# alexbuburuzan/MObI

Hardware: AMD Instinct MI355X
Metric: denoising throughput (UNet element-forwards/s = steps/s x UNet batch) (higher is better)
Workload: dtype bf16; 1 GPU; mobi_nusc_512 UNet denoising step, 8 objects/GPU (UNet batch 16), latent 64x64, DDIM-50 schedule, cfg_scale 1.0; objects_per_gpu=8, unet_batch=16, latent=64, sampler=ddim, parallelism=dp1 (objects sharded, no collective in the loop)

## Files before the change

### include/mobi_engine.h

```cpp
#ifndef MOBI_ENGINE_H_
#define MOBI_ENGINE_H_

#include <stddef.h>
#include <stdint.h>

#ifdef __cplusplus
extern "C" {
#endif

#define MOBI_ABI_VERSION 6

enum { MOBI_OK = 0, MOBI_ERR_ARG = -1, MOBI_ERR_UNSUPPORTED = -2, MOBI_ERR_LAUNCH = -3, MOBI_ERR_ALIGN = -4 };
enum { MOBI_F16 = 0, MOBI_BF16 = 1 };

int mobi_abi_version(void);
const char* mobi_error_string(int code);
size_t mobi_struct_size(int id);
int mobi_tuning_reload(void);
int mobi_build_info(void);

enum { MOBI_EPI_NONE = 0, MOBI_EPI_GEGLU = 1, MOBI_EPI_LEAKY_RELU = 2 };
enum { MOBI_OUT_ROWS = 0,
       MOBI_OUT_TRANSPOSED = 1,
       MOBI_OUT_ROWS_F32 = 2 };

typedef struct mobi_igemm_params {
  const void* src0;
  const void* src1;
  int32_t c0, c1;
  int32_t batch;
  int32_t hin, win;
  int32_t upsample;
  int32_t hout, wout;
  int32_t kh, kw, stride, pad_h, pad_w;
  int64_t src_img_stride;
  const void* weight;
  int32_t groups;
  int64_t w_group_stride;
  int32_t n_packed;
  int32_t cout;
  const float* bias;
  const float* rowvec;
  int32_t rowvec_stride;
  const void* residual;
  int64_t res_img_stride;
  void* out;
  int64_t out_img_stride;
  int32_t out_mode;
  int32_t epilogue;
  float scale;
  int32_t dtype;
  int32_t split_k;
  void* ws;
  int32_t k_order;
  const void* weight_tiled;
  void* sync;
  const float* ln_svec;
  float ln_eps;
  int32_t defer_finish;
} mobi_igemm_params;

int mobi_igemm(const mobi_igemm_params* p, void* stream);
int32_t mobi_igemm_slab_count(const mobi_igemm_params* p);
int mobi_igemm_finish(const mobi_igemm_params* p, void* stream);
int mobi_igemm_plan_splits(const mobi_igemm_params* p);
enum { MOBI_IGEMM_STAGED_128 = 0, MOBI_IGEMM_STAGED_256 = 1, MOBI_IGEMM_DIRECT_LDS = 2, MOBI_IGEMM_PINGPONG = 3,
       MOBI_IGEMM_RING_128 = 4, MOBI_IGEMM_RING_256 = 5, MOBI_IGEMM_RING_128W = 6, MOBI_IGEMM_SMALL = 7 };
int mobi_igemm_kernel_variant(const mobi_igemm_params* p);
size_t mobi_igemm_workspace_bytes(const mobi_igemm_params* p, int32_t splits);
size_t mobi_igemm_sync_bytes(const mobi_igemm_params* p, int32_t splits);

typedef struct mobi_split_source {
  const float* slabs;
  int32_t count;
  int32_t row_stride;
  const float* bias;
  const float* rowvec;
  int32_t rowvec_stride;
  const void* residual;
  int64_t res_img_stride;
  void* finished;
} mobi_split_source;

typedef struct mobi_groupnorm_params {
  const void* src0;
  const void* src1;
  int32_t c0, c1;
  int32_t batch, hw;
  const float* gamma;
  const float* beta;
  float eps;
  int32_t silu;
  void* out;
  void* ws;
  int32_t dtype;
  int32_t src_f32;
  int32_t out_mode;
  void* sync;
  const mobi_split_source* src0_split;
} mobi_groupnorm_params;

size_t mobi_groupnorm_workspace_bytes(int32_t batch, int32_t hw);
int mobi_groupnorm_takes_split(int32_t c0, int32_t c1, int32_t batch, int32_t hw);
int mobi_groupnorm(const mobi_groupnorm_params* p, void* stream);

typedef struct mobi_layernorm_params {
  const void* src; void* out;
  int32_t images, rows_per_image, channels;
  int64_t src_img_stride, out_img_stride;
  const float* gamma; const float* beta; float eps;
  int32_t dtype;
} mobi_layernorm_params;
int mobi_layernorm(const mobi_layernorm_params* p, void* stream);

typedef struct mobi_attention_params {
  const void* q;  int64_t q_img_stride;  int32_t q_row_stride;
  const void* k;  int64_t k_img_stride;  int32_t k_row_stride;
  const void* vt; int64_t vt_img_stride; int32_t vt_row_stride;
  void* out;      int64_t out_img_stride; int32_t out_row_stride;
  int32_t images, heads, dh, tq, tk;
  float scale;
// ... 335 lines not shown
```

### mobi_amd/_lib.py

```python
import ctypes as C
import os

HERE = os.path.dirname(os.path.abspath(__file__))
LIB_PATH = os.path.join(HERE, "libmobi_hip.so")

MOBI_F16, MOBI_BF16 = 0, 1
ABI_VERSION = 6
EPI_NONE, EPI_GEGLU, EPI_LEAKY_RELU = 0, 1, 2
OUT_ROWS, OUT_TRANSPOSED, OUT_ROWS_F32 = 0, 1, 2
ACT_NONE, ACT_SILU, ACT_GELU = 0, 1, 2

vp, i32, i64, f32 = C.c_void_p, C.c_int32, C.c_int64, C.c_float


class EngineUnavailable(RuntimeError):
    pass


class EngineError(RuntimeError):
    pass


class IgemmParams(C.Structure):
    _fields_ = [("src0", vp), ("src1", vp), ("c0", i32), ("c1", i32), ("batch", i32), ("hin", i32), ("win", i32),
# ... 131 lines not shown
    _fields_ = [("frames", vp), ("corners_xy", vp), ("invert", vp), ("crop", vp), ("gt", vp), ("inpaint", vp), ("mask", vp),
                ("batch", i32), ("H", i32), ("W", i32), ("height", i32), ("width", i32)]


class LpipsDistanceParams(C.Structure):
    _fields_ = [("feat", vp), ("lin", vp), ("out", vp), ("ws", vp), ("pairs", i32), ("hw", i32), ("channels", i32), ("eps", f32),
                ("relu_in_place", i32), ("dtype", i32)]


class ImageNormalizeParams(C.Structure):
    _fields_ = [("src", vp), ("out", vp), ("batch", i32), ("channels", i32), ("hw", i32), ("shift", f32 * 4), ("scale", f32 * 4),
                ("nhwc_channels", i32), ("dtype", i32)]


class MtTensor(C.Structure):
    _fields_ = [("param", vp), ("grad", vp), ("exp_avg", vp), ("exp_avg_sq", vp), ("n", i64)]


class MtPair(C.Structure):
    _fields_ = [("a", vp), ("b", vp), ("n", i64)]


MT_EMA, MT_SWAP = 0, 1


class MtChunk(C.Structure):
    _fields_ = [("offset", i64), ("tensor", i32), ("reserved", i32)]


class GradStatsRecord(C.Structure):
    _fields_ = [("sumsq", C.c_double), ("nonfinite", i32), ("reserved", i32)]


STRUCT_IDS = {0: IgemmParams, 1: GroupNormParams, 2: LayerNormParams, 3: AttentionParams, 4: CtxAttentionParams,
              5: SkinnyLinearParams, 6: ConvSmallCinParams, 7: ConvSmallCoutParams, 8: DdimStepParams, 9: TwoKeyAdapterParams,
              10: RangePasteParams, 11: LidarMetricsParams, 12: RangePrepareParams, 13: ImagePrepareParams,
              14: FfGegluParams, 15: RowChainParams, 16: ChainOp,
              17: LayerNormBwdParams, 18: AttentionBwdParams, 19: SplitSource, 20: DpmStepParams,
              21: LpipsDistanceParams, 22: ImageNormalizeParams, 23: MtTensor, 24: MtChunk, 25: GradStatsRecord,
              26: MtPair}

SYMBOLS = {
    "mobi_abi_version": (C.c_int, []),
    "mobi_error_string": (C.c_char_p, [C.c_int]),
    "mobi_struct_size": (C.c_size_t, [C.c_int]),
    "mobi_tuning_reload": (C.c_int, []),
    "mobi_build_info": (C.c_int, []),
    "mobi_igemm": (C.c_int, [C.POINTER(IgemmParams), vp]),
    "mobi_igemm_plan_splits": (C.c_int, [C.POINTER(IgemmParams)]),
    "mobi_igemm_kernel_variant": (C.c_int, [C.POINTER(IgemmParams)]),
    "mobi_igemm_workspace_bytes": (C.c_size_t, [C.POINTER(IgemmParams), i32]),
    "mobi_igemm_sync_bytes": (C.c_size_t, [C.POINTER(IgemmParams), i32]),
    "mobi_igemm_slab_count": (i32, [C.POINTER(IgemmParams)]),
    "mobi_igemm_finish": (C.c_int, [C.POINTER(IgemmParams), vp]),
    "mobi_groupnorm_takes_split": (C.c_int, [i32, i32, i32, i32]),
    "mobi_groupnorm_workspace_bytes": (C.c_size_t, [i32, i32]),
    "mobi_groupnorm": (C.c_int, [C.POINTER(GroupNormParams), vp]),
    "mobi_layernorm": (C.c_int, [C.POINTER(LayerNormParams), vp]),
    "mobi_attention": (C.c_int, [C.POINTER(AttentionParams), vp]),
    "mobi_ctx_attention": (C.c_int, [C.POINTER(CtxAttentionParams), vp]),
    "mobi_two_key_adapter": (C.c_int, [C.POINTER(TwoKeyAdapterParams), vp]),
    "mobi_two_key_adapter_fuses_ln": (C.c_int, [i32, i64]),
    "mobi_softmax_rows": (C.c_int, [vp, vp, i64, i32, i32, vp]),
    "mobi_skinny_linear": (C.c_int, [C.POINTER(SkinnyLinearParams), vp]),
    "mobi_layernorm_rows_f32": (C.c_int, [vp, vp, vp, vp, i32, i32, i32, i32, f32, vp]),
    "mobi_linear_f32": (C.c_int, [vp, vp, vp, vp, i32, i32, i32, i32, i32, i32, vp]),
    "mobi_ff_geglu": (C.c_int, [C.POINTER(FfGegluParams), vp]),
    "mobi_ff_geglu_packed_bytes": (C.c_size_t, [i32, i32]),
    "mobi_row_chain": (C.c_int, [C.POINTER(RowChainParams), vp]),
    "mobi_groupnorm_scale_shift": (C.c_int, [vp, vp, vp, f32, vp, vp, i32, i32, i32, i32, vp]),
    "mobi_row_chain_weight_bytes": (C.c_size_t, [i32]),
    "mobi_row_chain_supported": (C.c_int, [i32, i32]),
    "mobi_row_chain_adapter_image_bytes": (C.c_size_t, [i32]),
    "mobi_row_chain_adapter_image": (C.c_int, [vp, vp, vp, vp, i32, i32, i32, i32, vp, vp]),
    "mobi_trunk_add": (C.c_int, [vp, vp, vp, i64, i32, vp]),
    "mobi_split_f32": (C.c_int, [vp, vp, i64, i32, i32, i32, vp]),
    "mobi_transpose": (C.c_int, [vp, i64, vp, i32, i32, i32, vp]),
    "mobi_tile_weights": (C.c_int, [vp, vp, i32, i32, vp]),
    "mobi_backward_partial_blocks": (i32, [i64]),
    "mobi_colsum": (C.c_int, [vp, i64, i64, i32, i32, vp, vp, vp]),
    "mobi_layernorm_bwd": (C.c_int, [C.POINTER(LayerNormBwdParams), vp]),
    "mobi_geglu_fwd": (C.c_int, [vp, vp, i64, i32, i32, vp]),
    "mobi_geglu_bwd": (C.c_int, [vp, vp, vp, i64, i32, i32, vp]),
    "mobi_attention_bwd": (C.c_int, [C.POINTER(AttentionBwdParams), vp]),
    "mobi_groupnorm_bwd_workspace_floats": (C.c_size_t, [i32, i32, i32]),
    "mobi_groupnorm_bwd": (C.c_int, [vp, vp, vp, vp, f32, i32, vp, vp, i32, i32, i32, i32, vp, vp]),
    "mobi_sumpool2": (C.c_int, [vp, vp, i32, i32, i32, i32, i32, vp]),
    "mobi_add": (C.c_int, [vp, vp, vp, i64, i32, vp]),
    "mobi_silu_bwd_f32": (C.c_int, [vp, vp, vp, i64, vp]),
    "mobi_adamw_step": (C.c_int, [vp, vp, vp, vp, i64, f32, f32, f32, f32, f32, i32, vp]),
    "mobi_multi_tensor_workspace_bytes": (C.c_size_t, [C.POINTER(i32)]),
    "mobi_grad_stats": (C.c_int, [vp, i32, vp, i32, vp, vp, vp]),
    "mobi_adamw_multi": (C.c_int, [vp, i32, vp, i32, f32, f32, f32, f32, f32, f32, i32, vp]),
    "mobi_ema_multi": (C.c_int, [vp, i32, vp, i32, f32, i32, vp]),
    "mobi_quick_gelu": (C.c_int, [vp, vp, i64, i32, vp]),
    "mobi_timestep_embedding": (C.c_int, [vp, vp, vp, i32, i32, vp]),
    "mobi_conv_small_cin": (C.c_int, [C.POINTER(ConvSmallCinParams), vp]),
    "mobi_conv_small_cout": (C.c_int, [C.POINTER(ConvSmallCoutParams), vp]),
    "mobi_ddim_step": (C.c_int, [C.POINTER(DdimStepParams), vp]),
    "mobi_dpm_step": (C.c_int, [C.POINTER(DpmStepParams), vp]),
    "mobi_lincomb4": (C.c_int, [vp, vp, vp, vp, vp, f32, f32, f32, f32, i64, vp]),
    "mobi_q_sample": (C.c_int, [vp, vp, vp, vp, vp, vp, i32, i32, i32, vp]),
    "mobi_mask_blend": (C.c_int, [vp, vp, vp, vp, f32, f32, i32, i32, i32, vp]),
    "mobi_posterior_sample": (C.c_int, [vp, vp, vp, i32, i32, i32, i32, i32, f32, vp]),
    "mobi_range_denorm": (C.c_int, [vp, vp, vp, f32, f32, f32, f32, i32, i32, vp, vp, i32, i32, vp]),
    "mobi_range_paste": (C.c_int, [C.POINTER(RangePasteParams), vp]),
# ... 57 lines not shown
```

### mobi_amd/csrc/igemm.hip

```cpp
#include <stdlib.h>

#include <type_traits>

#include "common.h"
#include "tuning.h"
#include "igemm_small.h"

#ifndef MOBI_FRAG2
#define MOBI_FRAG2 0
#endif
#ifndef MOBI_DMA_KS
#define MOBI_DMA_KS 1
#endif
#if defined(MOBI_IGEMM_FENCE) && MOBI_IGEMM_FENCE
#define MOBI_SCHED_FENCE() __builtin_amdgcn_sched_barrier(0)
#else
#define MOBI_SCHED_FENCE() ((void)0)
#endif

#ifndef MOBI_DBG_SKIP
#define MOBI_DBG_SKIP 0
#endif
#ifndef MOBI_PP_DMA_KS
#define MOBI_PP_DMA_KS 1
// ... 1639 lines not shown
#pragma unroll
  for (int i = 0; i < 4; ++i) {
    sum = __builtin_amdgcn_fdot2(q.p[i], one, sum, false);
    sq = __builtin_amdgcn_fdot2(q.p[i], q.p[i], sq, false);
  }
}
__device__ __forceinline__ void rowstat_acc(const bf16x8& x, float& sum, float& sq) {
  struct Q { bf16x2_t p[4]; };
  const Q q = __builtin_bit_cast(Q, x);
  const bf16x2_t one = {(__bf16)1.0f, (__bf16)1.0f};
#pragma unroll
  for (int i = 0; i < 4; ++i) {
    sum = __builtin_amdgcn_fdot2_f32_bf16(q.p[i], one, sum, false);
    sq = __builtin_amdgcn_fdot2_f32_bf16(q.p[i], q.p[i], sq, false);
  }
}

template <int NT, int MT, int SPW>
__device__ __forceinline__ void ln_fold_acc(const IgemmArgs& a, f32x4 (&acc)[NT][MT], const float (&ls_sum)[SPW],
                                            const float (&ls_sq)[SPW], float* s_rowstat, int lane, int wm, int wn, int nw0,
                                            bool add_bias) {
  const int r16 = lane & 15, g4 = lane >> 4;
  const float inv_k = 1.0f / (float)a.ktot;
#pragma unroll
  for (int i = 0; i < SPW; ++i) {
    float sm = ls_sum[i], sq = ls_sq[i];
    sm += __shfl_xor(sm, 16, 64); sq += __shfl_xor(sq, 16, 64);
    sm += __shfl_xor(sm, 32, 64); sq += __shfl_xor(sq, 32, 64);
    const float mean = sm * inv_k;
    const float var = fmaxf(sq * inv_k - mean * mean, 0.f);
    if (g4 == 0) {
      float* d = s_rowstat + ((wm * MT + SPW * wn + i) * 16 + r16) * 2;
      d[0] = mean; d[1] = rsqrtf(var + a.ln_eps);
    }
  }
  __syncthreads();
#pragma unroll
  for (int ni = 0; ni < NT; ++ni) {
    const int n = nw0 + ni * 16 + g4 * 4;
    f32x4 sv = f32x4{0.f, 0.f, 0.f, 0.f}, bv = f32x4{0.f, 0.f, 0.f, 0.f};
    if (n < a.n_packed) {
      sv = *reinterpret_cast<const f32x4*>(a.ln_svec + n);
      if (add_bias && a.bias) bv = *reinterpret_cast<const f32x4*>(a.bias + n);
    }
#pragma unroll
    for (int mi = 0; mi < MT; ++mi) {
      const float* d = s_rowstat + ((wm * MT + mi) * 16 + r16) * 2;
      const float mean = d[0], rstd = d[1];
      acc[ni][mi] = rstd * (acc[ni][mi] - mean * sv) + bv;
    }
  }
}

template <typename T, int NT, bool TR, int NW, int MT, bool LNF = false, bool LEAKY = false>
__global__ __launch_bounds__(NW * 64, 2) void igemm_ring_kernel(const IgemmArgs a) {
  typedef typename Vec8<T>::type frag_t;
  constexpr bool WIDE = NW == 8;
  constexpr int BM = 2 * MT * 16;
  constexpr int APW = BM / 16 / NW;
  constexpr int WAVE_N = NT * 16;
  constexpr int BN = (NW / 2) * WAVE_N;
  constexpr int WPIECES = BN / 16;
  constexpr int SLOT = (BM + BN) * 64;
  constexpr int RING = 4 * SLOT;
  constexpr int STAGE_BYTES = EpiGeom<32, TR, NT>::BYTES;
  constexpr int LDS_BYTES = RING > NW * STAGE_BYTES ? RING : NW * STAGE_BYTES;
  constexpr unsigned OOB = 0x80000000u;
  __shared__ __attribute__((aligned(16))) unsigned char lds[LDS_BYTES];
  __shared__ int s_arrive;
  __shared__ float s_rowstat[LNF ? BM * 2 : 2];
  static_assert(!(LNF && TR), "the LayerNorm fold has no transposed-output form");
  typedef __attribute__((address_space(3))) void* lds_ptr_t;

  const int tid = threadIdx.x, lane = tid & 63, wave = tid >> 6;
  const int wave_s = __builtin_amdgcn_readfirstlane(wave);
  const int wm = wave & 1, wn = wave >> 1;
  const int group = blockIdx.z;
  const int nblk = a.tiles_m * a.tiles_n;
  const int L = xcd_remap(blockIdx.x, nblk);
  MOBI_TILE_OF(L, tile_m, tile_n);
  const int m0 = tile_m * BM, n0 = tile_n * BN;
  constexpr int SPW = MT / (NW / 2);
  constexpr bool lnf = LNF;
  float ls_sum[SPW], ls_sq[SPW];
#pragma unroll
  for (int i = 0; i < SPW; ++i) ls_sum[i] = ls_sq[i] = 0.f;
  MOBI_STAMP_AT(0);
  const bool w_tiled = a.w_tiled != nullptr;
  const T* wgt = (w_tiled ? reinterpret_cast<const T*>(a.w_tiled) : reinterpret_cast<const T*>(a.weight)) + (long long)group * a.w_group_stride;
  const __amdgpu_buffer_rsrc_t rx0 = __builtin_amdgcn_make_buffer_rsrc(const_cast<void*>(a.src0), 0, a.src0_bytes, 0x00020000);
  const __amdgpu_buffer_rsrc_t rx1 =
      __builtin_amdgcn_make_buffer_rsrc(const_cast<void*>(a.src1 ? a.src1 : a.src0), 0, a.src1 ? a.src1_bytes : 0, 0x00020000);
  const __amdgpu_buffer_rsrc_t rw = __builtin_amdgcn_make_buffer_rsrc(const_cast<T*>(wgt), 0, a.w_bytes, 0x00020000);

  const int rp = lane >> 2;
  const unsigned perm = (0x1320u >> (((rp >> 2) & 3) * 4)) & 3u;
  const unsigned chunk16 = (((unsigned)lane & 3u) ^ perm) * 16u;
  int x_base[APW], x_h[APW], x_w[APW];
  bool x_ok[APW];
#pragma unroll
  for (int j = 0; j < APW; ++j) {
    const int m = m0 + 16 * (APW * wave + j) + rp;
    x_ok[j] = m < a.M;
    const int mm = x_ok[j] ? m : 0;
    const int img = mm / a.hw_out, rem = mm - img * a.hw_out;
    const int ho = rem / a.wout, wo = rem - ho * a.wout;
    x_base[j] = (group * a.imgs_per_group + img) * a.img_pix_stride;
    x_h[j] = ho * a.stride - a.pad_h;
    x_w[j] = wo * a.stride - a.pad_w;
  }
  unsigned w_off[3];
#pragma unroll
  for (int i = 0; i < 3; ++i) {
    const int piece = wave + NW * i;
    const int n = n0 + 16 * piece + rp;
    w_off[i] = (piece < WPIECES && n < a.n_packed) ? (unsigned)n * (unsigned)a.ktot * 2u + chunk16 : OOB;
    if (w_tiled) w_off[i] = (piece < WPIECES && n0 + 16 * piece < a.n_packed)
                                ? (unsigned)(n0 / 16 + piece) * (unsigned)(a.ktot >> 5) * 1024u + (unsigned)lane * 16u : OOB;
  }
  const int hlog = a.hin << a.up, wlog = a.win << a.up;
  const int ks_all = a.ktot >> 5;
  const int ks_begin = blockIdx.y * a.nk_per * 2;
  const int ks_end = min(ks_all, ks_begin + a.nk_per * 2);
  int u_c, u_tap, u_ky, u_kx;
  {
    const long long c_first = (long long)ks_begin * 32;
    u_tap = (int)(c_first / a.C); u_c = (int)(c_first - (long long)u_tap * a.C);
    u_ky = u_tap / a.kw; u_kx = u_tap - u_ky * a.kw;
  }
  unsigned f_row[APW];
#pragma unroll
  for (int j = 0; j < APW; ++j) f_row[j] = OOB;
  int f_tap = -1, f_src = -1, f_ks = ks_begin;

  auto issue_step = [&]() {
    unsigned char* st = lds + (f_ks & 3) * SLOT;
    const bool live = f_ks < ks_end;
    const int src = u_c >= a.c0 ? 1 : 0;
    if (live && (u_tap != f_tap || src != f_src)) {
      f_tap = u_tap; f_src = src;
      const unsigned cs2 = (unsigned)(src ? a.c1 : a.c0) * 2u;
#pragma unroll
      for (int j = 0; j < APW; ++j) {
        const int hi = x_h[j] + u_ky, wi = x_w[j] + u_kx;
        const bool ok = x_ok[j] && (unsigned)hi < (unsigned)hlog && (unsigned)wi < (unsigned)wlog;
        f_row[j] = ok ? (unsigned)(x_base[j] + (hi >> a.up) * a.win + (wi >> a.up)) * cs2 + chunk16 : OOB;
      }
    }
    const int soff = (src ? u_c - a.c0 : u_c) * 2;
#pragma unroll
    for (int j = 0; j < APW; ++j) {
      const unsigned vo = live ? f_row[j] : OOB;
      if (src) __builtin_amdgcn_raw_ptr_buffer_load_lds(rx1, (lds_ptr_t)(st + 16 * (APW * wave_s + j) * 64), 16, vo, soff, 0, 0);
      else     __builtin_amdgcn_raw_ptr_buffer_load_lds(rx0, (lds_ptr_t)(st + 16 * (APW * wave_s + j) * 64), 16, vo, soff, 0, 0);
    }
    const int kb = w_tiled ? f_ks * 1024 : f_ks * 64;
#pragma unroll
    for (int i = 0; i < 3; ++i) {
      if (i == 2 && (NT != 5 || wave_s >= NW / 2)) break;
      const unsigned vo = live ? w_off[i] : OOB;
      __builtin_amdgcn_raw_ptr_buffer_load_lds(rw, (lds_ptr_t)(st + BM * 64 + (wave_s + NW * i) * 1024), 16, vo, kb, 0, 0);
    }
    ++f_ks;
    if (live) {
      u_c += 32;
      if (u_c >= a.C) { u_c = 0; ++u_tap; if (++u_kx == a.kw) { u_kx = 0; ++u_ky; } }
    }
  };
  auto wait_step = [&]() {
    if (NT == 5 && wave_s < NW / 2) {
      if (APW == 2) asm volatile("s_waitcnt vmcnt(10)" ::: "memory"); else asm volatile("s_waitcnt vmcnt(8)" ::: "memory");
    } else {
      if (APW == 2) asm volatile("s_waitcnt vmcnt(8)" ::: "memory"); else asm volatile("s_waitcnt vmcnt(6)" ::: "memory");
    }
  };

  f32x4 acc[NT][MT];
#pragma unroll
  for (int i = 0; i < NT; ++i)
#pragma unroll
    for (int j = 0; j < MT; ++j) acc[i][j] = f32x4{0.f, 0.f, 0.f, 0.f};

  const int r16 = lane & 15, g4 = lane >> 4;
  if constexpr (WIDE && MT == 8 && !TR) {
    if (!lnf && a.ring_direct && (a.bias || a.rowvec)) {
      const float* vec = a.bias;
      if (a.rowvec) {
        const int img = __builtin_amdgcn_readfirstlane((m0 + wm * 128) / a.hw_out);
        vec = a.rowvec + (long long)(group * a.imgs_per_group + img) * a.rowvec_stride;
      }
#pragma unroll
      for (int i = 0; i < NT; ++i) {
        const f32x4 b = *reinterpret_cast<const f32x4*>(vec + n0 + wn * WAVE_N + i * 16 + g4 * 4);
#pragma unroll
        for (int j = 0; j < MT; ++j) acc[i][j] = b;
      }
    }
  }
  const unsigned fsw = (((unsigned)g4 ^ ((0x1320u >> (((r16 >> 2) & 3) * 4)) & 3u)) << 4);
  const unsigned char* xrd = lds + (wm * MT * 16 + r16) * 64 + fsw;
  const unsigned char* wrd = lds + BM * 64 + (wn * WAVE_N + r16) * 64 + fsw;

  auto read_frags = [&](int s, frag_t (&xf)[MT], frag_t (&wf)[NT]) {
    const int so = (s & 3) * SLOT;
#pragma unroll
    for (int mi = 0; mi < MT; ++mi) xf[mi] = __builtin_bit_cast(frag_t, ld16(xrd + so + mi * 16 * 64));
#pragma unroll
    for (int ni = 0; ni < NT; ++ni) wf[ni] = __builtin_bit_cast(frag_t, ld16(wrd + so + ni * 16 * 64));
  };
  auto multiply = [&](const frag_t (&xf)[MT], const frag_t (&wf)[NT]) {
    __builtin_amdgcn_s_setprio(1);
#pragma unroll
    for (int ni = 0; ni < NT; ++ni)
#pragma unroll
      for (int mi = 0; mi < MT; ++mi)
        acc[ni][mi] = TR ? mfma16(xf[mi], wf[ni], acc[ni][mi]) : mfma16(wf[ni], xf[mi], acc[ni][mi]);
    __builtin_amdgcn_s_setprio(0);
  };
  auto multiply_stats = [&](const frag_t (&xf)[MT], const frag_t (&wf)[NT], auto wnc) {
    constexpr int WNC = decltype(wnc)::value;
    __builtin_amdgcn_s_setprio(1);
#pragma unroll
    for (int ni = 0; ni < NT; ++ni)
#pragma unroll
      for (int mi = 0; mi < MT; ++mi) {
        acc[ni][mi] = TR ? mfma16(xf[mi], wf[ni], acc[ni][mi]) : mfma16(wf[ni], xf[mi], acc[ni][mi]);
        if (ni == 0 && mi < SPW) rowstat_acc(xf[SPW * WNC + mi], ls_sum[mi], ls_sq[mi]);
      }
#pragma unroll
    for (int i = 0; i < 8 * SPW; ++i) {
      __builtin_amdgcn_sched_group_barrier(0x008, 2, 0);
      __builtin_amdgcn_sched_group_barrier(0x002, 1, 0);
    }
#pragma unroll
    for (int i = 0; i < SPW; ++i) asm volatile("" : "+v"(ls_sum[i]), "+v"(ls_sq[i]));
    __builtin_amdgcn_s_setprio(0);
  };
#define MOBI_RING_BARRIER()                   \
  do {                                        \
    __builtin_amdgcn_sched_barrier(0);        \
    __builtin_amdgcn_s_barrier();             \
    __builtin_amdgcn_sched_barrier(0);        \
  } while (0)

  issue_step(); issue_step(); issue_step();
  auto k_loop = [&](auto wnc) {
  if constexpr (WIDE && MOBI_RING_STAGGER) {
    const bool late = wave_s >= NW / 2;
    wait_step();
    MOBI_STAMP_AT(1);
    if (late) MOBI_RING_BARRIER();
#if MOBI_STAMP == 4
    unsigned long long wp_t[8], wp_acc[7] = {0, 0, 0, 0, 0, 0, 0};
#define MOBI_WP(i) wp_t[i] = __builtin_amdgcn_s_memtime()
#else
#define MOBI_WP(i) ((void)0)
// ... 24 lines not shown
#if MOBI_STAMP == 4
      MOBI_WP(7);
      if (s > ks_begin) for (int i = 0; i < 7; ++i) wp_acc[i] += wp_t[i + 1] - wp_t[i];
#endif
    }
#if MOBI_STAMP == 4
    if (g_phase && lane == 0) {
      unsigned long long* d = g_phase + ((size_t)(blockIdx.x + gridDim.x * (blockIdx.y + gridDim.y * blockIdx.z)) * 8 + wave) * 8;
      for (int i = 0; i < 7; ++i) d[i] = wp_acc[i];
      d[7] = (unsigned long long)(ks_end - ks_begin - 1);
    }
#endif
#undef MOBI_WP
    if (!late) MOBI_RING_BARRIER();
  } else {
#if MOBI_STAMP == 4
    unsigned long long rp_t[6], rp_acc[5] = {0, 0, 0, 0, 0};
#define MOBI_RP(i) rp_t[i] = __builtin_amdgcn_s_memtime()
#else
#define MOBI_RP(i) ((void)0)
#endif
#pragma clang loop unroll(disable)
    for (int s = ks_begin; s < ks_end; ++s) {
      MOBI_RP(0);
      wait_step();
      MOBI_RP(1);
      MOBI_RING_BARRIER();
      MOBI_RP(2);
      frag_t xf[MT], wf[NT];
      read_frags(s, xf, wf);
      __builtin_amdgcn_sched_barrier(0);
      issue_step();
      __builtin_amdgcn_sched_barrier(0);
      MOBI_RP(3);
      asm volatile("s_waitcnt lgkmcnt(0)" ::: "memory");
      MOBI_RP(4);
      if constexpr (lnf) multiply_stats(xf, wf, wnc); else multiply(xf, wf);
#if MOBI_STAMP == 4
      asm volatile("s_nop 0" ::: "memory");
      MOBI_RP(5);
      if (s > ks_begin) for (int i = 0; i < 5; ++i) rp_acc[i] += rp_t[i + 1] - rp_t[i];
#endif
    }
#if MOBI_STAMP == 4
    if (g_phase && lane == 0) {
      unsigned long long* d = g_phase + ((size_t)(blockIdx.x + gridDim.x * (blockIdx.y + gridDim.y * blockIdx.z)) * 8 + wave) * 8;
      for (int i = 0; i < 5; ++i) d[i] = rp_acc[i];
      d[5] = (unsigned long long)(ks_end - ks_begin - 1);
    }
#endif
#undef MOBI_RP
  }
  };
  if constexpr (lnf) {
    const int wn_s = wave_s >> 1;
    if (wn_s == 0) k_loop(std::integral_constant<int, 0>{});
    else if (wn_s == 1 || NW == 4) k_loop(std::integral_constant<int, 1>{});
    else if (wn_s == 2) k_loop(std::integral_constant<int, NW == 8 ? 2 : 0>{});
    else k_loop(std::integral_constant<int, NW == 8 ? 3 : 0>{});
  } else {
    k_loop(std::integral_constant<int, 0>{});
  }
#undef MOBI_RING_BARRIER
  MOBI_STAMP_AT(2);
  if constexpr (lnf) {
    ln_fold_acc<NT, MT, SPW>(a, acc, ls_sum, ls_sq, s_rowstat, lane, wm, wave_s >> 1, n0 + wn * WAVE_N,
                             WIDE && MT == 8 && a.ring_direct);
  }
  if constexpr (MT == 4 && !TR && !LEAKY) {
    if (a.sm_direct) {
      asm volatile("s_waitcnt vmcnt(0)" ::: "memory");
      const int nw0 = n0 + wn * WAVE_N, mw0 = m0 + wm * 64;
      if (a.split_ws) {
        float* wsp = a.split_ws + (long long)blockIdx.y * a.M * a.n_packed;
#pragma unroll
        for (int mi = 0; mi < 4; ++mi) {
          float* rowp = wsp + (long long)(mw0 + mi * 16 + r16) * a.n_packed + nw0 + g4 * 4;
#pragma unroll
          for (int ni = 0; ni < NT; ++ni) slab_store16(a.sync_mode == 1, rowp + ni * 16, __builtin_bit_cast(u32x4, acc[ni][mi]));
        }
        if (a.sync) {
          splitk_arrive_and_finish<T, NW * 64>(a, tile_m * a.tiles_n + tile_n, m0, BM, n0, BN, &s_arrive);
        }
      } else {
        DirectEpiRegs<NT> q;
#pragma unroll
        for (int ni = 0; ni < NT; ++ni) { q.bias[ni] = u32x4{0u, 0u, 0u, 0u}; q.res[ni][0] = q.res[ni][1] = u32x4{0u, 0u, 0u, 0u}; }
        direct_epilogue_request<T, NT>(a, q, lane, group, nw0, mw0);
        asm volatile("s_waitcnt vmcnt(0)" ::: "memory");
        if (a.epilogue == MOBI_EPI_GEGLU) direct_epilogue<T, NT, true>(a, acc, q, lane, group, nw0, mw0);
        else direct_epilogue<T, NT, false>(a, acc, q, lane, group, nw0, mw0);
      }
      return;
    }
  }
  if constexpr (WIDE && MT == 8 && !TR && !LEAKY) {
    if (a.ring_direct) {
      asm volatile("s_waitcnt vmcnt(0)" ::: "memory");
      if constexpr (MT == 8) {
        if (a.epilogue == MOBI_EPI_GEGLU) ring_register_epilogue<T, NT, true>(a, acc, lane, group, n0 + wn * WAVE_N, m0 + wm * 128);
        else ring_register_epilogue<T, NT, false>(a, acc, lane, group, n0 + wn * WAVE_N, m0 + wm * 128);
      }
#if MOBI_STAMP
      asm volatile("s_waitcnt vmcnt(0)" ::: "memory");
      MOBI_STAMP_AT(3);
      if (g_stamps && threadIdx.x == 0) {
        unsigned long long* d = g_stamps + (size_t)(blockIdx.x + gridDim.x * (blockIdx.y + gridDim.y * blockIdx.z)) * 8;
        unsigned hw, xcc;
        asm volatile("s_getreg_b32 %0, hwreg(HW_REG_HW_ID)" : "=s"(hw));
        asm volatile("s_getreg_b32 %0, hwreg(HW_REG_XCC_ID)" : "=s"(xcc));
        d[4] = ((unsigned long long)xcc << 32) | hw;
        d[5] = (unsigned long long)(ks_end - ks_begin);
        d[6] = 1;
      }
#endif
// ... 277 lines not shown
      for (int j = 0; j < 4; ++j) { o[j] += v0[j]; o[4 + j] += v1[j]; }
    }
    const int img = m / a.hw_out, rem = m - img * a.hw_out;
    if (a.bias) {
      float bb[8];
      ld8f(a.bias + n, bb);
#pragma unroll
      for (int j = 0; j < 8; ++j) o[j] += bb[j];
    }
    if (a.rowvec) {
      float rv[8];
      ld8f(a.rowvec + (long long)img * a.rowvec_stride + n, rv);
#pragma unroll
      for (int j = 0; j < 8; ++j) o[j] += rv[j];
    }
    if (resid) {
      float rf[8];
      unpack8<T>(ld16(resid + (long long)img * a.res_img_stride + (long long)rem * a.cout + n), rf);
#pragma unroll
      for (int j = 0; j < 8; ++j) o[j] += rf[j];
    }
    const long long off = (long long)img * a.out_img_stride + (long long)rem * a.cout + n;
    if (a.out_mode == MOBI_OUT_ROWS_F32) {
      *reinterpret_cast<f32x4*>(outF + off) = f32x4{o[0], o[1], o[2], o[3]};
      *reinterpret_cast<f32x4*>(outF + off + 4) = f32x4{o[4], o[5], o[6], o[7]};
    } else {
      st16(outT + off, pack8<T>(o));
    }
  }
}

static int compute_units() {
  if (tuning().persist_blocks > 0) return tuning().persist_blocks;
  static int cached[64] = {0};
  int dev = 0;
  if (hipGetDevice(&dev) != hipSuccess || dev < 0 || dev >= 64) return 256;
  if (!cached[dev]) {
    int n = 0;
    if (hipDeviceGetAttribute(&n, hipDeviceAttributeMultiprocessorCount, dev) != hipSuccess || n <= 0) n = 256;
    cached[dev] = n;
  }
  return cached[dev];
}

template <typename T>
static int launch_splitk_reduce(const IgemmArgs& a, hipStream_t st) {
  long long blocks = ((long long)a.M * (a.cout >> 3) + 255) / 256;
  if (blocks > 4096) blocks = 4096;
  hipLaunchKernelGGL((igemm_splitk_reduce_kernel<T>), dim3((unsigned)blocks), dim3(256), 0, st, a);
  MOBI_CHECK_LAUNCH();
  return MOBI_OK;
}

template <typename T>
static int launch_igemm(const mobi_igemm_params* p, const IgemmArgs& a, int groups, hipStream_t st) {
  const bool tr = p->out_mode == MOBI_OUT_TRANSPOSED;
  const bool nt5 = (a.n_packed % 160) == 0;
  dim3 grid(a.tiles_m * a.tiles_n, a.splits, groups);
#define MOBI_IGEMM_LAUNCH(NT_, TR_, WM_, FAST_) \
  hipLaunchKernelGGL((igemm_kernel<T, NT_, TR_, WM_, FAST_>), grid, dim3(128 * WM_), 0, st, a)
#ifdef MOBI_DEV
#define MOBI_IGEMM_BY_FAST(NT_, TR_, WM_) \
  do { if (a.fast) MOBI_IGEMM_LAUNCH(NT_, TR_, WM_, true); else MOBI_IGEMM_LAUNCH(NT_, TR_, WM_, false); } while (0)
#else
#define MOBI_IGEMM_BY_FAST(NT_, TR_, WM_) MOBI_IGEMM_LAUNCH(NT_, TR_, WM_, false)
#endif
#define MOBI_IGEMM_BY_TR(NT_, WM_) \
  do { if (tr) MOBI_IGEMM_BY_FAST(NT_, true, WM_); else MOBI_IGEMM_BY_FAST(NT_, false, WM_); } while (0)
  if (a.epilogue == MOBI_EPI_LEAKY_RELU) {
    if (a.wide == 2) {
      if (nt5) hipLaunchKernelGGL((igemm_ring_kernel<T, 5, false, 8, 8, false, true>), grid, dim3(512), 0, st, a);
      else     hipLaunchKernelGGL((igemm_ring_kernel<T, 4, false, 8, 8, false, true>), grid, dim3(512), 0, st, a);
    } else {
      if (nt5) hipLaunchKernelGGL((igemm_ring_kernel<T, 5, false, 4, 4, false, true>), grid, dim3(256), 0, st, a);
      else     hipLaunchKernelGGL((igemm_ring_kernel<T, 4, false, 4, 4, false, true>), grid, dim3(256), 0, st, a);
    }
  }
  else if (a.wide == 2) {
#define MOBI_W2_LAUNCH(NT_, TR_) hipLaunchKernelGGL((igemm_ring_kernel<T, NT_, TR_, 8, 8>), grid, dim3(512), 0, st, a)
    if (a.ln_svec) {
      if (nt5) hipLaunchKernelGGL((igemm_ring_kernel<T, 5, false, 8, 8, true>), grid, dim3(512), 0, st, a);
      else     hipLaunchKernelGGL((igemm_ring_kernel<T, 4, false, 8, 8, true>), grid, dim3(512), 0, st, a);
    }
    else if (nt5) { if (tr) MOBI_W2_LAUNCH(5, true); else MOBI_W2_LAUNCH(5, false); }
    else     { if (tr) MOBI_W2_LAUNCH(4, true); else MOBI_W2_LAUNCH(4, false); }
#undef MOBI_W2_LAUNCH
  }
  else if (a.wide == 1) {
    if (nt5) hipLaunchKernelGGL((igemm_ring_kernel<T, 5, false, 8, 4>), grid, dim3(512), 0, st, a);
    else     hipLaunchKernelGGL((igemm_ring_kernel<T, 4, false, 8, 4>), grid, dim3(512), 0, st, a);
  }
  else if (a.wm == 4 && a.fast && a.glds && a.pp) {
    dim3 block(512);
    dim3 pgrid(grid.x < (unsigned)compute_units() ? grid.x : (unsigned)compute_units(), grid.y, grid.z);
    if (a.split_ws) {
      if (nt5) hipLaunchKernelGGL((igemm_pp_kernel<T, 5, false, true>), pgrid, block, 0, st, a);
      else     hipLaunchKernelGGL((igemm_pp_kernel<T, 4, false, true>), pgrid, block, 0, st, a);
    } else {
#define MOBI_PP_LAUNCH(NT_, G_) hipLaunchKernelGGL((igemm_pp_kernel<T, NT_, G_>), pgrid, block, 0, st, a)
      if (a.epilogue == MOBI_EPI_GEGLU) { if (nt5) MOBI_PP_LAUNCH(5, true); else MOBI_PP_LAUNCH(4, true); }
      else                              { if (nt5) MOBI_PP_LAUNCH(5, false); else MOBI_PP_LAUNCH(4, false); }
#undef MOBI_PP_LAUNCH
    }
  }
#ifdef MOBI_DEV
  else if (a.wm == 4 && a.fast && a.glds) {
    dim3 block(512);
    dim3 pgrid(grid.x < (unsigned)compute_units() ? grid.x : (unsigned)compute_units(), grid.y, grid.z);
    const int mode = tr ? 1 : (a.epi_direct ? (a.epilogue == MOBI_EPI_GEGLU ? 3 : 2) : 0);
#define MOBI_GLDS_LAUNCH(NT_, MODE_) hipLaunchKernelGGL((igemm_glds_kernel<T, NT_, MODE_>), pgrid, block, 0, st, a)
#define MOBI_GLDS_BY_MODE(NT_)                                                                     \
// ... 298 lines not shown
  }
  a.small = lnf || leaky ? 0 : small_tile(p);
  if (lnf && !(a.wide || a.sm)) return MOBI_ERR_UNSUPPORTED;
  a.sync = nullptr; a.sync_mode = 0;
  if (a.split_ws && p->sync && !a.small && tuning().fused_split != 0 && a.splits <= 4 &&
      (long long)a.splits * a.M * a.n_packed * 4 < 0x7fffffffLL) {
    if (reinterpret_cast<uintptr_t>(p->sync) & 3) return MOBI_ERR_ALIGN;
    const long long tiles = (long long)a.tiles_m * a.tiles_n;
    const bool pp_launch = !a.wide && a.wm == 4 && a.fast && a.glds && a.pp;
    const bool ring_launch = a.wide || a.sm;
    const int mode = tuning().fused_split == 1 ? 1 : 2;
    if ((ring_launch || (pp_launch && tiles <= (long long)compute_units())) && (mode == 1 || tiles % 8 == 0)) {
      a.sync = reinterpret_cast<int*>(p->sync);
      a.sync_mode = mode;
    }
  }
  return MOBI_OK;
}

static int launch_small(const mobi_igemm_params* p, const mobi::IgemmArgs& a, hipStream_t st) {
  mobi::SmallGemmArgs s;
  s.src0 = a.src0; s.src1 = a.src1; s.c0 = a.c0; s.c1 = a.c1;
  s.taps = a.kh * a.kw; s.hin = a.hin; s.win = a.win;
  s.hw = a.hw_out; s.img_pix_stride = a.img_pix_stride;
  s.weight = a.weight;
  s.M = a.M; s.N = a.n_packed; s.K = a.ktot;
  s.bias = a.bias; s.rowvec = a.rowvec; s.rowvec_stride = a.rowvec_stride;
  s.residual = a.residual; s.res_img_stride = a.res_img_stride;
  s.out = a.out; s.out_img_stride = a.out_img_stride; s.out_f32 = a.out_mode == MOBI_OUT_ROWS_F32;
  s.scale = a.scale;
  s.tiles_m = (a.M + a.small - 1) / a.small; s.tiles_n = a.n_packed / a.small;
  const long long wbytes = (long long)a.n_packed * a.ktot * 2, abytes = (long long)a.M * a.ktot * 2;
  s.n_major = wbytes > abytes;
  return mobi::launch_small_gemm(s, p->dtype, st);
}

extern "C" int mobi_igemm(const mobi_igemm_params* p, void* stream) {
  using namespace mobi;
  IgemmArgs a;
  const int rc = igemm_prepare(p, a);
  if (rc != MOBI_OK) return rc;
  hipStream_t st = reinterpret_cast<hipStream_t>(stream);
  if (a.small) return launch_small(p, a, st);
  return p->dtype == MOBI_F16 ? launch_igemm<f16_t>(p, a, p->groups, st) : launch_igemm<bf16_t>(p, a, p->groups, st);
}

extern "C" int32_t mobi_igemm_slab_count(const mobi_igemm_params* p) {
  mobi::IgemmArgs a;
  const int rc = igemm_prepare(p, a);
  if (rc != MOBI_OK) return rc;
  return a.small ? 1 : a.splits;
}

extern "C" int mobi_igemm_finish(const mobi_igemm_params* p, void* stream) {
  using namespace mobi;
  IgemmArgs a;
  const int rc = igemm_prepare(p, a);
  if (rc != MOBI_OK) return rc;
  if (!a.split_ws || a.small || a.sync) return MOBI_ERR_ARG;
  hipStream_t st = reinterpret_cast<hipStream_t>(stream);
  return p->dtype == MOBI_F16 ? launch_splitk_reduce<f16_t>(a, st) : launch_splitk_reduce<bf16_t>(a, st);
}

extern "C" int mobi_igemm_kernel_variant(const mobi_igemm_params* p) {
  mobi::IgemmArgs a;
  const int rc = igemm_prepare(p, a);
  if (rc != MOBI_OK) return rc;
  if (a.small) return MOBI_IGEMM_SMALL;
  if (a.wide) return a.wide == 2 ? MOBI_IGEMM_RING_256 : MOBI_IGEMM_RING_128W;
  if (a.wm == 4 && a.fast && a.glds) return a.pp ? MOBI_IGEMM_PINGPONG : MOBI_IGEMM_DIRECT_LDS;
  if (a.wm == 4) return MOBI_IGEMM_STAGED_256;
  return a.sm ? MOBI_IGEMM_RING_128 : MOBI_IGEMM_STAGED_128;
}
```

### mobi_amd/csrc/tuning.h

```cpp
#pragma once
namespace mobi {
struct Tuning {
  int persist_blocks;
  int pp_split;
  int wm;
  int fast;
  int glds;
  int lin;
  int epi_direct;
  int pp;
  int sm;
  int wide;
  int wide128;
  int ring_direct;
  int sm_direct;
  int w_tiled;
  int n_major;
  int sm64;
  int split_target;
  int fused_split;
  int split_longk;
  int split_round4;
  int attn_bwd_exact_d;
  int small;
  int small_mflop;
  int small_conv_m;
  int tka_mfma;
  int attn_nw;
  int attn_sp;
  int tka_rows;
  int attn_nw8_blocks;
  int attn_h16;
  int attn_xcd;
  int cout_mfma;
  int skinny_mfma;
  int gn_coop;
  int gn_fused;
  int gn_split_pw4;
  int attn_v3;
};
const Tuning& tuning();
}
```

### mobi_amd/csrc/tuning.hip

```cpp
#include <atomic>
#include <cstdlib>
#include <mutex>

#include "common.h"
#include "tuning.h"

namespace mobi {
namespace {
Tuning g_tuning;
std::once_flag g_once;

int env_int(const char* name) {
  const char* e = getenv(name);
  return (e && e[0]) ? atoi(e) : -1;
}
void read_env() {
  g_tuning.persist_blocks = env_int("MOBI_IGEMM_PERSIST_BLOCKS");
  g_tuning.pp_split = env_int("MOBI_IGEMM_PP_SPLIT");
  g_tuning.wm = env_int("MOBI_IGEMM_WM");
  g_tuning.fast = env_int("MOBI_IGEMM_FAST");
  g_tuning.glds = env_int("MOBI_IGEMM_GLDS");
  g_tuning.lin = env_int("MOBI_IGEMM_LIN");
  g_tuning.epi_direct = env_int("MOBI_IGEMM_EPI_DIRECT");
  g_tuning.pp = env_int("MOBI_IGEMM_PP");
  g_tuning.sm = env_int("MOBI_IGEMM_SM");
  g_tuning.wide = env_int("MOBI_IGEMM_WIDE");
  g_tuning.wide128 = env_int("MOBI_IGEMM_WIDE128");
  g_tuning.ring_direct = env_int("MOBI_IGEMM_RING_DIRECT");
  g_tuning.sm_direct = env_int("MOBI_IGEMM_SM_DIRECT");
  g_tuning.w_tiled = env_int("MOBI_IGEMM_WTILED");
  g_tuning.sm64 = env_int("MOBI_IGEMM_SM64");
  g_tuning.n_major = env_int("MOBI_IGEMM_N_MAJOR");
  g_tuning.split_target = env_int("MOBI_IGEMM_SPLIT_TARGET");
  g_tuning.split_longk = env_int("MOBI_IGEMM_SPLIT_LONGK");
  g_tuning.split_round4 = env_int("MOBI_IGEMM_SPLIT_ROUND4");
  g_tuning.attn_bwd_exact_d = env_int("MOBI_ATTN_BWD_EXACT_D");
  g_tuning.fused_split = env_int("MOBI_IGEMM_FUSED_SPLIT");
  g_tuning.small = env_int("MOBI_IGEMM_SMALL");
  g_tuning.small_mflop = env_int("MOBI_IGEMM_SMALL_MFLOP");
  g_tuning.small_conv_m = env_int("MOBI_IGEMM_SMALL_CONV_M");
  g_tuning.tka_mfma = env_int("MOBI_TKA_MFMA");
  g_tuning.attn_nw = env_int("MOBI_ATTN_NW");
  g_tuning.attn_sp = env_int("MOBI_ATTN_SP");
  g_tuning.attn_v3 = env_int("MOBI_ATTN_V3");
  g_tuning.gn_fused = env_int("MOBI_GN_FUSED");
  g_tuning.gn_coop = env_int("MOBI_GN_COOP");
  g_tuning.gn_split_pw4 = env_int("MOBI_GN_SPLIT_PW4");
  g_tuning.skinny_mfma = env_int("MOBI_SKINNY_MFMA");
  g_tuning.cout_mfma = env_int("MOBI_COUT_MFMA");
  g_tuning.attn_xcd = env_int("MOBI_ATTN_XCD");
  g_tuning.attn_h16 = env_int("MOBI_ATTN_H16");
  g_tuning.attn_nw8_blocks = env_int("MOBI_ATTN_NW8_BLOCKS");
  g_tuning.tka_rows = env_int("MOBI_TKA_ROWS");
}
}

const Tuning& tuning() {
  std::call_once(g_once, read_env);
  return g_tuning;
}
}

extern "C" int mobi_tuning_reload(void) {
  std::call_once(mobi::g_once, [] {});
  mobi::read_env();
  return MOBI_OK;
}

extern "C" int mobi_build_info(void) {
#ifdef MOBI_DEV
  return 1;
#else
  return 0;
#endif
}
```

Baseline: 838.9 UNet element-forwards/s.

## Add persistent tile-walk mode to the wide ring igemm kernel

Adds a PERSIST variant of the 256-pixel ring implicit-GEMM kernel that launches one block per compute unit. Each block walks several output tiles and prefetches the next tile's operands into the LDS ring while the current tile's epilogue runs. It applies when the tile count exceeds the CU count and K is modest (or when forced by env), removing per-tile launch/ramp overhead and overlapping epilogue with loads. In exchange it adds register pressure and complex ring-index bookkeeping, and it loses the load balance of a normal oversubscribed grid.

```diff
diff --git a/include/mobi_engine.h b/include/mobi_engine.h
--- a/include/mobi_engine.h
+++ b/include/mobi_engine.h
@@ -67,6 +67,7 @@
 enum { MOBI_IGEMM_STAGED_128 = 0, MOBI_IGEMM_STAGED_256 = 1, MOBI_IGEMM_DIRECT_LDS = 2, MOBI_IGEMM_PINGPONG = 3,
        MOBI_IGEMM_RING_128 = 4, MOBI_IGEMM_RING_256 = 5, MOBI_IGEMM_RING_128W = 6, MOBI_IGEMM_SMALL = 7 };
 int mobi_igemm_kernel_variant(const mobi_igemm_params* p);
+int32_t mobi_igemm_persistent_supported(const mobi_igemm_params* p);
 size_t mobi_igemm_workspace_bytes(const mobi_igemm_params* p, int32_t splits);
 size_t mobi_igemm_sync_bytes(const mobi_igemm_params* p, int32_t splits);
 
diff --git a/mobi_amd/_lib.py b/mobi_amd/_lib.py
--- a/mobi_amd/_lib.py
+++ b/mobi_amd/_lib.py
@@ -207,6 +207,7 @@
     "mobi_igemm_workspace_bytes": (C.c_size_t, [C.POINTER(IgemmParams), i32]),
     "mobi_igemm_sync_bytes": (C.c_size_t, [C.POINTER(IgemmParams), i32]),
     "mobi_igemm_slab_count": (i32, [C.POINTER(IgemmParams)]),
+    "mobi_igemm_persistent_supported": (i32, [C.POINTER(IgemmParams)]),
     "mobi_igemm_finish": (C.c_int, [C.POINTER(IgemmParams), vp]),
     "mobi_groupnorm_takes_split": (C.c_int, [i32, i32, i32, i32]),
     "mobi_groupnorm_workspace_bytes": (C.c_size_t, [i32, i32]),
diff --git a/mobi_amd/csrc/igemm.hip b/mobi_amd/csrc/igemm.hip
--- a/mobi_amd/csrc/igemm.hip
+++ b/mobi_amd/csrc/igemm.hip
@@ -1715,8 +1715,9 @@
   }
 }
 
-template <typename T, int NT, bool TR, int NW, int MT, bool LNF = false, bool LEAKY = false>
+template <typename T, int NT, bool TR, int NW, int MT, bool LNF = false, bool LEAKY = false, bool PERSIST = false>
 __global__ __launch_bounds__(NW * 64, 2) void igemm_ring_kernel(const IgemmArgs a) {
+  static_assert(!PERSIST || (NW == 8 && MT == 8 && !TR && !LEAKY), "tile walk: 256-pixel register-epilogue launches only");
   typedef typename Vec8<T>::type frag_t;
   constexpr bool WIDE = NW == 8;
   constexpr int BM = 2 * MT * 16;
@@ -1795,12 +1796,56 @@
 #pragma unroll
   for (int j = 0; j < APW; ++j) f_row[j] = OOB;
   int f_tap = -1, f_src = -1, f_ks = ks_begin;
-
+  int f_bid = blockIdx.x, f_ring = 0;
+
+  auto set_fetch_tile = [&](int fm0, int fn0, int t) {
+    const int ln = t & 63, wv = t >> 6, rp_t = ln >> 2;
+    const unsigned ck = (((unsigned)ln & 3u) ^ ((0x1320u >> (((rp_t >> 2) & 3) * 4)) & 3u)) * 16u;
+#pragma unroll
+    for (int j = 0; j < APW; ++j) {
+      const int m = fm0 + 16 * (APW * wv + j) + rp_t;
+      const int img = m >> a.hw_shift, rem = m & (a.hw_out - 1);
+      if constexpr (LNF) {
+        f_row[j] = (unsigned)(img * a.img_pix_stride + rem) * ((unsigned)a.c0 * 2u) + ck;
+      } else {
+        x_ok[j] = true;
+        x_base[j] = img * a.img_pix_stride;
+        x_h[j] = (rem >> a.w_shift) * a.stride - a.pad_h;
+        x_w[j] = (rem & (a.wout - 1)) * a.stride - a.pad_w;
+      }
+    }
+#pragma unroll
+    for (int i = 0; i < 3; ++i) {
+      const int piece = wv + NW * i;
+      w_off[i] = piece < WPIECES ? (unsigned)(fn0 + 16 * piece + rp_t) * (unsigned)a.ktot * 2u + ck : OOB;
+      if (w_tiled) w_off[i] = piece < WPIECES ? (unsigned)(fn0 / 16 + piece) * (unsigned)(a.ktot >> 5) * 1024u + (unsigned)ln * 16u : OOB;
+    }
+  };
+  if constexpr (PERSIST && LNF) {
+#pragma unroll
+    for (int j = 0; j < APW; ++j) f_row[j] = (unsigned)(x_base[j] + x_h[j] * a.win + x_w[j]) * ((unsigned)a.c0 * 2u) + chunk16;
+  }
+  auto next_fetch_tile = [&]() {
+    if (f_ks == ks_end && f_bid + (int)gridDim.x < nblk) {
+      f_bid += (int)gridDim.x;
+      const int Lf = xcd_remap(f_bid, nblk);
+      MOBI_TILE_OF(Lf, ftm, ftn);
+      int t = tid;
+      asm volatile("" : "+v"(t));
+      set_fetch_tile(ftm * BM, ftn * BN, t);
+      f_ks = ks_begin; f_tap = -1; f_src = -1;
+      u_c = 0; u_tap = 0; u_ky = 0; u_kx = 0;
+    }
+  };
   auto issue_step = [&]() {
-    unsigned char* st = lds + (f_ks & 3) * SLOT;
+    if constexpr (PERSIST) next_fetch_tile();
+    int f_slot = f_ks;
+    if constexpr (PERSIST) f_slot = f_ring;
+    unsigned char* st = lds + (f_slot & 3) * SLOT;
     const bool live = f_ks < ks_end;
-    const int src = u_c >= a.c0 ? 1 : 0;
-    if (live && (u_tap != f_tap || src != f_src)) {
+    int src = u_c >= a.c0 ? 1 : 0;
+    if constexpr (PERSIST && LNF) src = 0;
+    if (!(PERSIST && LNF) && live && (u_tap != f_tap || src != f_src)) {
       f_tap = u_tap; f_src = src;
       const unsigned cs2 = (unsigned)(src ? a.c1 : a.c0) * 2u;
 #pragma unroll
@@ -1825,6 +1870,7 @@
       __builtin_amdgcn_raw_ptr_buffer_load_lds(rw, (lds_ptr_t)(st + BM * 64 + (wave_s + NW * i) * 1024), 16, vo, kb, 0, 0);
     }
     ++f_ks;
+    if constexpr (PERSIST) ++f_ring;
     if (live) {
       u_c += 32;
       if (u_c >= a.C) { u_c = 0; ++u_tap; if (++u_kx == a.kw) { u_kx = 0; ++u_ky; } }
@@ -1860,11 +1906,28 @@
       }
     }
   }
+  auto start_sums = [&](int tm0, int tn0, int t) {
+    const int wm_t = (t >> 6) & 1, wn_t = t >> 7, g4_t = (t & 63) >> 4;
+    const float* vec = a.bias;
+    if (a.rowvec) {
+      const int img = __builtin_amdgcn_readfirstlane((tm0 + wm_t * 128) >> a.hw_shift);
+      vec = a.rowvec + (long long)img * a.rowvec_stride;
+    }
+#pragma unroll
+    for (int i = 0; i < NT; ++i) {
+      f32x4 b = f32x4{0.f, 0.f, 0.f, 0.f};
+      if (!lnf && vec) b = *reinterpret_cast<const f32x4*>(vec + tn0 + wn_t * WAVE_N + i * 16 + g4_t * 4);
+#pragma unroll
+      for (int j = 0; j < MT; ++j) acc[i][j] = b;
+    }
+  };
   const unsigned fsw = (((unsigned)g4 ^ ((0x1320u >> (((r16 >> 2) & 3) * 4)) & 3u)) << 4);
   const unsigned char* xrd = lds + (wm * MT * 16 + r16) * 64 + fsw;
   const unsigned char* wrd = lds + BM * 64 + (wn * WAVE_N + r16) * 64 + fsw;
 
+  int c_ring = 0;
   auto read_frags = [&](int s, frag_t (&xf)[MT], frag_t (&wf)[NT]) {
+    if constexpr (PERSIST) s += c_ring;
     const int so = (s & 3) * SLOT;
 #pragma unroll
     for (int mi = 0; mi < MT; ++mi) xf[mi] = __builtin_bit_cast(frag_t, ld16(xrd + so + mi * 16 * 64));
@@ -1995,15 +2058,45 @@
 #undef MOBI_RP
   }
   };
-  if constexpr (lnf) {
-    const int wn_s = wave_s >> 1;
-    if (wn_s == 0) k_loop(std::integral_constant<int, 0>{});
-    else if (wn_s == 1 || NW == 4) k_loop(std::integral_constant<int, 1>{});
-    else if (wn_s == 2) k_loop(std::integral_constant<int, NW == 8 ? 2 : 0>{});
-    else k_loop(std::integral_constant<int, NW == 8 ? 3 : 0>{});
-  } else {
-    k_loop(std::integral_constant<int, 0>{});
-  }
+#define MOBI_RING_BY_WN(f_)                                                       \
+  if constexpr (lnf) {                                                            \
+    const int wn_s = wave_s >> 1;                                                 \
+    if (wn_s == 0) f_(std::integral_constant<int, 0>{});                          \
+    else if (wn_s == 1 || NW == 4) f_(std::integral_constant<int, 1>{});          \
+    else if (wn_s == 2) f_(std::integral_constant<int, NW == 8 ? 2 : 0>{});       \
+    else f_(std::integral_constant<int, NW == 8 ? 3 : 0>{});                      \
+  } else {                                                                        \
+    f_(std::integral_constant<int, 0>{});                                         \
+  }
+  if constexpr (PERSIST) {
+    auto tile_walk = [&](auto wnc) {
+      for (int c_bid = blockIdx.x, tm0 = m0, tn0 = n0;;) {
+        k_loop(wnc);
+        int t = tid;
+        asm volatile("" : "+v"(t));
+        const int lane_t = t & 63, wm_t = (t >> 6) & 1, wn_t = lnf ? decltype(wnc)::value : t >> 7;
+        if constexpr (lnf) ln_fold_acc<NT, MT, SPW>(a, acc, ls_sum, ls_sq, s_rowstat, lane_t, wm_t, wn_t, tn0 + wn_t * WAVE_N, true);
+        asm volatile("s_waitcnt vmcnt(0)" ::: "memory");
+        if (a.epilogue == MOBI_EPI_GEGLU) ring_register_epilogue<T, NT, true>(a, acc, lane_t, 0, tn0 + wn_t * WAVE_N, tm0 + wm_t * 128);
+        else ring_register_epilogue<T, NT, false>(a, acc, lane_t, 0, tn0 + wn_t * WAVE_N, tm0 + wm_t * 128);
+        c_bid += (int)gridDim.x;
+        if (c_bid >= nblk) break;
+        const int Lc = xcd_remap(c_bid, nblk);
+        MOBI_TILE_OF(Lc, ctm, ctn);
+        tm0 = ctm * BM; tn0 = ctn * BN;
+        c_ring += ks_end - ks_begin;
+        set_fetch_tile(tm0, tn0, t);
+        f_tap = -1;
+        start_sums(tm0, tn0, t);
+#pragma unroll
+        for (int i = 0; i < SPW; ++i) ls_sum[i] = ls_sq[i] = 0.f;
+      }
+    };
+    MOBI_RING_BY_WN(tile_walk)
+    return;
+  }
+  MOBI_RING_BY_WN(k_loop)
+#undef MOBI_RING_BY_WN
 #undef MOBI_RING_BARRIER
   MOBI_STAMP_AT(2);
   if constexpr (lnf) {
@@ -2387,11 +2480,31 @@
   return MOBI_OK;
 }
 
+static int ring_persist_grid(const IgemmArgs& a, int groups) {
+  if (a.small || a.wide != 2 || a.splits != 1 || groups != 1 || !a.ring_direct || a.epilogue == MOBI_EPI_LEAKY_RELU ||
+      a.out_mode != MOBI_OUT_ROWS || (a.ktot >> 5) < 3 || a.hw_shift < 0 || a.w_shift < 0 || (a.ln_svec && (a.pad_h || a.pad_w)) ||
+      tuning().ring_persist == 0)
+    return 0;
+  if (tuning().ring_persist != 1 && a.ktot >= 1280) return 0;
+  const long long tiles = (long long)a.tiles_m * a.tiles_n;
+  return tiles > (long long)compute_units() ? compute_units() : 0;
+}
+
 template <typename T>
 static int launch_igemm(const mobi_igemm_params* p, const IgemmArgs& a, int groups, hipStream_t st) {
   const bool tr = p->out_mode == MOBI_OUT_TRANSPOSED;
   const bool nt5 = (a.n_packed % 160) == 0;
   dim3 grid(a.tiles_m * a.tiles_n, a.splits, groups);
+  if (const int pg = ring_persist_grid(a, groups)) {
+    const dim3 pgrid(pg);
+#define MOBI_W2P_LAUNCH(NT_, LNF_) \
+  hipLaunchKernelGGL((igemm_ring_kernel<T, NT_, false, 8, 8, LNF_, false, true>), pgrid, dim3(512), 0, st, a)
+    if (a.ln_svec) { if (nt5) MOBI_W2P_LAUNCH(5, true); else MOBI_W2P_LAUNCH(4, true); }
+    else           { if (nt5) MOBI_W2P_LAUNCH(5, false); else MOBI_W2P_LAUNCH(4, false); }
+#undef MOBI_W2P_LAUNCH
+    MOBI_CHECK_LAUNCH();
+    return MOBI_OK;
+  }
 #define MOBI_IGEMM_LAUNCH(NT_, TR_, WM_, FAST_) \
   hipLaunchKernelGGL((igemm_kernel<T, NT_, TR_, WM_, FAST_>), grid, dim3(128 * WM_), 0, st, a)
 #ifdef MOBI_DEV
@@ -2796,6 +2909,18 @@
   return a.small ? 1 : a.splits;
 }
 
+extern "C" int32_t mobi_igemm_persistent_supported(const mobi_igemm_params* p) {
+  using namespace mobi;
+  IgemmArgs a;
+  const int rc = igemm_prepare(p, a);
+  if (rc != MOBI_OK) return rc;
+  if (a.small) return 0;
+  const long long tiles = (long long)a.tiles_m * a.tiles_n;
+  if (a.epilogue != MOBI_EPI_LEAKY_RELU && !a.wide && a.wm == 4 && a.fast && a.glds && a.pp)
+    return tiles > (long long)compute_units() ? compute_units() : 0;
+  return ring_persist_grid(a, p->groups);
+}
+
 extern "C" int mobi_igemm_finish(const mobi_igemm_params* p, void* stream) {
   using namespace mobi;
   IgemmArgs a;
diff --git a/mobi_amd/csrc/tuning.h b/mobi_amd/csrc/tuning.h
--- a/mobi_amd/csrc/tuning.h
+++ b/mobi_amd/csrc/tuning.h
@@ -14,6 +14,7 @@
   int wide128;
   int ring_direct;
   int sm_direct;
+  int ring_persist;
   int w_tiled;
   int n_major;
   int sm64;
diff --git a/mobi_amd/csrc/tuning.hip b/mobi_amd/csrc/tuning.hip
--- a/mobi_amd/csrc/tuning.hip
+++ b/mobi_amd/csrc/tuning.hip
@@ -28,6 +28,7 @@
   g_tuning.wide128 = env_int("MOBI_IGEMM_WIDE128");
   g_tuning.ring_direct = env_int("MOBI_IGEMM_RING_DIRECT");
   g_tuning.sm_direct = env_int("MOBI_IGEMM_SM_DIRECT");
+  g_tuning.ring_persist = env_int("MOBI_IGEMM_RING_PERSIST");
   g_tuning.w_tiled = env_int("MOBI_IGEMM_WTILED");
   g_tuning.sm64 = env_int("MOBI_IGEMM_SM64");
   g_tuning.n_major = env_int("MOBI_IGEMM_N_MAJOR");
```

Result: no change. 840.8 UNet element-forwards/s, median of 6 (+0.2%).
